# mrmod/h264decode

Hardware: AMD Instinct MI355X
Metric: 1080p Main CABAC frames/sec (higher is better)
Workload: dtype u8; 1 GPU; 1920x1080 Main CABAC IPPP GOP-30, 256 independent streams per GPU (32 distinct, each used 8 times), QP 28, 1 slice/frame, 1 ref; parallelism=streams sharded, no collective

## Files before the change

h264decode_amd/csrc/k_entropy.hip:

```cpp
#include <hip/hip_runtime.h>
#include "mi_kernels.h"
#include "k_common.h"

#ifndef MI_ENT_ISLICE_PRIO
#define MI_ENT_ISLICE_PRIO 0
#endif
#ifndef MI_ENT_MINWAVES
#define MI_ENT_MINWAVES 6
#endif
#ifndef MI_ENT_B
#define MI_ENT_B 0
#endif
#ifndef MI_ENT_FMO
#define MI_ENT_FMO MI_ENT_B
#endif
#ifndef MI_ENT_CABAC
#define MI_ENT_CABAC 0
#endif
#if MI_ENT_CABAC
#define ENT_CABAC(e) 1
#define IF_CAVLC(x) 0
#else
#define ENT_CABAC(e) ((e).cabac)
#define IF_CAVLC(x) (x)
#endif
#if MI_ENT_B
#define NL 2
#define MI_ENT_KERNEL k_entropy_b
#elif MI_ENT_FMO
#define NL 1
#define MI_ENT_KERNEL k_entropy_f
#elif MI_ENT_CABAC
#define NL 1
#define MI_ENT_KERNEL k_entropy_c
#else
#define NL 1
#define MI_ENT_KERNEL k_entropy
#endif
#define LANE (e.lane)
#define FI __device__ __forceinline__
#define LDS_SYNC()                                             \
    do {                                                       \
        __builtin_amdgcn_fence(__ATOMIC_RELEASE, "wavefront"); \
        __builtin_amdgcn_wave_barrier();                       \
        __builtin_amdgcn_fence(__ATOMIC_ACQUIRE, "wavefront"); \
    } while (0)

struct TopInfo {
    uint8_t type, t8x8, cbp, chroma_mode, cbf_dc;
    uint8_t dmask;
    uint16_t row;
    int8_t ipm[4];
    uint8_t nnz[8];
    int8_t ref[2][2];
    int16_t mv[NL][4][2];
    uint8_t mvd[NL][4][2];
};
#define TOP_DW (static_cast<int>(sizeof(TopInfo) / 4))
static_assert(sizeof(TopInfo) == (MI_ENT_B ? 72 : 48), "TopInfo layout");

struct Shared {
    uint8_t ctx[464];
#if !MI_ENT_CABAC
    uint8_t posmap[4][64];
#endif
    int16_t coef[MI_COEF_PER_MB];
    MbRec rec;
    TopInfo nb[4];
    int8_t ipm_c[32];
    uint8_t nnz_c[32];
    uint8_t nnzc_c[2][12];
    int8_t ref_c[NL][32];
    int8_t refi_c[NL][32];
    alignas(4) int16_t mv_c[NL][32][2];
    alignas(2) uint8_t mvd_c[NL][32][2];
    uint16_t parts[16];
    int8_t refs8[2][4];
    int8_t sub_type[4];
    uint8_t cur_cbf_dc, pad[3];
    int16_t ref_slot[NL][MI_MAX_REFS];
    uint32_t skip_tmpl[32];
    uint32_t role[64];
#if !MI_ENT_CABAC
    uint16_t vlc[MI_VLC_N];
#endif
    uint8_t coded[64];
#if MI_ENT_B
    uint32_t col[20];
    alignas(4) int16_t dmv[2][16][2];
    int8_t dref[2][4];
    int16_t dsf[MI_MAX_REFS];
#endif
};
#define GI(bx, by) (((by) + 1) * 6 + (bx) + 1)
enum { NB_LEFT = 0, NB_TL = 1, NB_TOP = 2 };

struct Ent {
    int lane;
    Shared *s;
    TopInfo *top;
    uint32_t pre_top;
    const DevTables *tab;
    const uint32_t *rbsp32;
    const SliceDesc *sd;
    const PicDesc *pd;
    MbRec *mbrec;
    int16_t *coefs;
    uint32_t *pool_head;
    uint32_t pool_blocks;
    uint32_t coef_cur, coef_end;
    uint64_t bitbuf;
    int bcnt;
    uint32_t wpos, wbase, rbsp_words;
    uint32_t win, winn, winx;
    uint32_t range, value;
    int avail;
    uint32_t ca, cb, wk;
    int wk_cat;
    uint32_t wk_c0;
    int wk_home;
    int wk_valid;
    uint32_t v_rlps, v_trans;
    uint32_t v_maps;
    uint32_t v_pos;
    uint32_t v_cat0, v_cat1;
    uint32_t v_qpc, v_refslot;
    uint32_t v_step;
    uint32_t aw, bw;
    int v_ipm;
    int qp, prev_dqp_nz, mbx, mby, cur_type, err;
    uint32_t qpw0, qpw1;
    int cabac, islice, wmb, hmb;
    int mono;
    int cip, t8x8_mode, cqp_off0, cqp_off1, nref;
    uint64_t mb_base;
#if MI_ENT_B
    int nref1, direct_spatial, d8inf, col_short, direct8;
    const uint32_t *col;
    uint32_t v_col;
    MbMv1 *mbmv1;
#endif
#if MI_ENT_STATS
    uint32_t bins;
    uint64_t tacc[4], tmark;
#endif
};
#if MI_ENT_STATS
#define MI_BINS(e) ((e).bins)
#define MI_COUNT_BIN(e) ((e).bins++)
#define MI_TT0(e) ((e).tmark = __builtin_readcyclecounter())
#define MI_TT(e, k) do { const uint64_t now_ = __builtin_readcyclecounter(); (e).tacc[k] += now_ - (e).tmark; (e).tmark = now_; } while (0)
#if MI_ENT_STATS == 4
#define MI_T0(e) ((void)0)
#define MI_T(e, k) ((void)0)
#define MI_R0(e) ((void)0)
#define MI_R(e, k) ((void)0)
#define MI_S(e, k) MI_TT(e, k)
#elif MI_ENT_STATS == 2
#define MI_T0(e) ((void)0)
#define MI_T(e, k) ((void)0)
#define MI_R0(e) ((void)0)
#define MI_R(e, k) ((void)0)
#define MI_R0(e) MI_TT0(e)
#define MI_R(e, k) MI_TT(e, k)
#else
#define MI_T0(e) MI_TT0(e)
#define MI_T(e, k) MI_TT(e, k)
#define MI_R0(e) ((void)0)
#define MI_R(e, k) ((void)0)
#endif
#else
#define MI_BINS(e) 0u
#define MI_COUNT_BIN(e) ((void)0)
#define MI_T0(e) ((void)0)
#define MI_T(e, k) ((void)0)
#define MI_R0(e) ((void)0)
#define MI_R(e, k) ((void)0)
#endif
#ifndef MI_S
#define MI_S(e, k) ((void)0)
#endif
#define RFL(x) __builtin_amdgcn_readfirstlane(x)
#define RDL(v, i) static_cast<uint32_t>(__builtin_amdgcn_readlane(static_cast<int>(v), static_cast<int>(i)))
extern "C" __device__ int mi_writelane(int val, int lane, int old) __asm("llvm.amdgcn.writelane.i32");

FI uint32_t cat_word0(int c) {
    const uint32_t maxnum[6] = {16, 15, 16, 4, 15, 64}, cbf[6] = {85, 89, 93, 97, 101, 64}, lim[6] = {4, 4, 4, 3, 4, 4}, pm[6] = {0, 1, 0, 3, 1, 2};
    const uint32_t nlast[6] = {15, 14, 15, 3, 14, 9};
    c = c < 6 ? c : 0;
    return maxnum[c] | (cbf[c] - 64) << 8 | lim[c] << 16 | pm[c] << 20 | nlast[c] << 24;
}
FI uint32_t cat_word1(int c, int field) {
    const uint32_t sig[6] = {105, 120, 134, 149, 152, 402}, last[6] = {166, 181, 195, 210, 213, 417}, ab[6] = {227, 237, 247, 257, 266, 426};
    const uint32_t sigf[6] = {277, 292, 306, 321, 324, 436}, lastf[6] = {338, 353, 367, 382, 385, 451};
    c = c < 6 ? c : 0;
    return (field ? sigf[c] : sig[c]) | (field ? lastf[c] : last[c]) << 10 | ab[c] << 20;
}

FI uint32_t load_win(const Ent &e, uint32_t base) {
    const uint32_t i = base + LANE;
    return i < e.rbsp_words ? __builtin_bswap32(e.rbsp32[i]) : 0u;
}
FI uint32_t fetch_word(Ent &e) {
    const uint32_t idx = e.wpos - e.wbase;
    e.wpos++;
    const uint32_t w0 = RDL(e.win, idx), w1 = RDL(e.winn, idx), w2 = RDL(e.winx, idx);
    return idx < 64 ? w0 : (idx < 128 ? w1 : w2);
}
FI void slide_window(Ent &e) {
    while (e.wpos - e.wbase >= 64) {
        e.win = e.winn, e.winn = e.winx;
        e.wbase += 64;
        e.winx = load_win(e, e.wbase + 128);
    }
}
FI uint32_t bitpos(const Ent &e) { return e.wpos * 32 - static_cast<uint32_t>(e.bcnt); }
FI void seek(Ent &e, uint32_t pos) {
// ... 718 lines not shown
            *reinterpret_cast<uint32_t *>(s->mv_c[0][g]) = w0, *reinterpret_cast<uint32_t *>(s->mv_c[1][g]) = w1;
        } else {
            *reinterpret_cast<uint32_t *>(s->dmv[0][l]) = w0, *reinterpret_cast<uint32_t *>(s->dmv[1][l]) = w1;
        }
        if (!((bx | by) & 1)) {
            if (commit)
                s->refs8[0][q] = static_cast<int8_t>(ref0), s->refs8[1][q] = static_cast<int8_t>(ref1);
            else
                s->dref[0][q] = static_cast<int8_t>(ref0), s->dref[1][q] = static_cast<int8_t>(ref1);
        }
    }
    LDS_SYNC();
}
FI void commit_direct(Ent &e, const int L, int q) {
    Shared *s = e.s;
    const int l = LANE, bx = l & 3, by = (l >> 2) & 3;
    if (l < 16 && (by >> 1) * 2 + (bx >> 1) == q) {
        const int g = GI(bx, by);
        s->ref_c[L][g] = s->dref[L][q];
        *reinterpret_cast<uint32_t *>(s->mv_c[L][g]) = *reinterpret_cast<const uint32_t *>(s->dmv[L][l]);
        if (!((bx | by) & 1)) s->refs8[L][q] = s->dref[L][q];
    }
    LDS_SYNC();
}
#endif

FI void read_ref_idx(Ent &e, const int L, int bx, int by, int w, int h, int nref) {
    Shared *s = e.s;
    int ref = 0;
    if (nref > 1) {
        if (ENT_CABAC(e)) {
            int ctx = (s->refi_c[L][GI(bx - 1, by)] > 0) + 2 * (s->refi_c[L][GI(bx, by - 1)] > 0);
            while (BIN_A(e, 54 + ctx)) {
                ctx = (ctx >> 2) + 4;
                if (++ref > 31) {
                    e.err = 3;
                    break;
                }
            }
        } else
            ref = IF_CAVLC(nref == 2 ? !get_bit(e) : static_cast<int>(get_ue(e)));
        if (ref >= nref || ref >= MI_MAX_REFS) e.err = 13, ref = 0;
    }
    {
        const int l = LANE, x = l & 3, y = (l >> 2) & 3;
        if (l < 16 && x >= bx && x < bx + w && y >= by && y < by + h) {
            s->refi_c[L][GI(x, y)] = static_cast<int8_t>(ref);
            if (!((x | y) & 1)) s->refs8[L][(y >> 1) * 2 + (x >> 1)] = static_cast<int8_t>(ref);
        }
        LDS_SYNC();
    }
}
FI void read_mv(Ent &e, const int L, int p) {
    Shared *s = e.s;
    const int bx = p & 3, by = (p >> 2) & 3, w = ((p >> 4) & 3) + 1, h = ((p >> 6) & 3) + 1, shape = (p >> 8) & 7;
    const int ref = s->refs8[L][(by >> 1) * 2 + (bx >> 1)];
    int d[2];
    for (int comp = 0; comp < 2; comp++) {
        int v;
        if (ENT_CABAC(e)) {
            const int sum = s->mvd_c[L][GI(bx - 1, by)][comp] + s->mvd_c[L][GI(bx, by - 1)][comp];
            const int base = comp ? 47 : 40;
            v = 0;
            if (BIN_A(e, base + (sum > 2) + (sum > 32))) {
                int ctx = base + 3;
                v = 1;
                while (v < 9 && BIN_A(e, ctx)) {
                    if (v < 4) ctx++;
                    v++;
                }
                if (v >= 9) v += cabac_egk(e, 3);
                if (cabac_bypass(e)) v = -v;
            }
        } else
            v = IF_CAVLC(get_se(e));
        d[comp] = v;
    }
    int px, py;
    predict_mv(e, L, bx, by, w, ref, shape, px, py);
    set_part(e, L, bx, by, w, h, ref, px + d[0], py + d[1], d[0], d[1]);
}

#if !MI_ENT_B
FI void pskip_fast(Ent &e) {
    Shared *s = e.s;
    int l = LANE;
    OPAQUE(l);
    const uint32_t *nbw = reinterpret_cast<const uint32_t *>(s->nb);
    const uint32_t tA = e.aw, tB = e.bw, tC = nbw[(NB_TOP + 1) * TOP_DW], tD = nbw[NB_TL * TOP_DW];
    const uint32_t rA = nbw[NB_LEFT * TOP_DW + 5], rB = nbw[NB_TOP * TOP_DW + 5], rC = nbw[(NB_TOP + 1) * TOP_DW + 5], rD = nbw[NB_TL * TOP_DW + 5];
    const uint32_t mA = nbw[NB_LEFT * TOP_DW + 6], mB = nbw[NB_TOP * TOP_DW + 6], mC = nbw[(NB_TOP + 1) * TOP_DW + 6], mD = nbw[NB_TL * TOP_DW + 9];
    auto ref_of = [](uint32_t t, uint32_t r, int byte) {
        const int type = static_cast<int>(t & 255u);
        return type == MBT_NONE ? -2 : (MB_IS_INTER(type) ? static_cast<int>(static_cast<int8_t>((r >> (8 * byte)) & 255u)) : -1);
    };
    auto mv_of = [](uint32_t t, uint32_t m) { return MB_IS_INTER(static_cast<int>(t & 255u)) ? m : 0u; };
    const int ra = ref_of(tA, rA, 0), rb = ref_of(tB, rB, 0);
    const bool c_ok = e.mbx + 1 < e.wmb && (tC & 255u) != MBT_NONE;
    const int rc = c_ok ? ref_of(tC, rC, 0) : ref_of(tD, rD, 1);
    const uint32_t va = mv_of(tA, mA), vb = mv_of(tB, mB), vc = c_ok ? mv_of(tC, mC) : mv_of(tD, mD);
    uint32_t mvw = 0;
    const bool zero = ra == -2 || rb == -2 || (ra == 0 && va == 0) || (rb == 0 && vb == 0);
    if (!zero) {
        const int na = ra == 0, nb_ = rb == 0, nc = rc == 0;
        if (na + nb_ + nc == 1)
            mvw = na ? va : (nb_ ? vb : vc);
        else {
            const int ax = static_cast<int16_t>(va & 0xffffu), ay = static_cast<int32_t>(va) >> 16, bx = static_cast<int16_t>(vb & 0xffffu), by = static_cast<int32_t>(vb) >> 16;
            const int cx = static_cast<int16_t>(vc & 0xffffu), cy = static_cast<int32_t>(vc) >> 16;
            mvw = (static_cast<uint32_t>(median3(ax, bx, cx)) & 0xffffu) | (static_cast<uint32_t>(median3(ay, by, cy)) << 16);
        }
    }
    e.cur_type = MBT_PSKIP;
    e.prev_dqp_nz = 0;
    if (l < TOP_DW) {
        const uint32_t row = MI_ENT_FMO ? static_cast<uint32_t>(e.mby + 1) << 16 : 0u;
        const uint32_t nw = l == 0 ? static_cast<uint32_t>(MBT_PSKIP) : (l == 1 ? row : (l == 2 ? 0xFFFFFFFFu : ((l >= 6 && l < 10) ? mvw : 0u)));
        uint32_t *tl = reinterpret_cast<uint32_t *>(&s->nb[NB_TL]), *tp = reinterpret_cast<uint32_t *>(&s->nb[NB_TOP]), *tr = reinterpret_cast<uint32_t *>(&s->nb[NB_TOP + 1]);
        const uint32_t old_top = tp[l], w1 = tr[l];
        tl[l] = old_top;
        tp[l] = w1;
        tr[l] = e.pre_top;
        reinterpret_cast<uint32_t *>(&s->nb[NB_LEFT])[l] = nw;
        reinterpret_cast<uint32_t *>(e.top + e.mbx)[l] = nw;
        e.pre_top = top_load(e, e.mbx + 3, l);
    } else if (l >= 32) {
        const int k = l - 32;
        const uint32_t t = s->skip_tmpl[k];
        const uint32_t w = k == 0 ? (static_cast<uint32_t>(MBT_PSKIP) | e.qpw0) : (k == 1 ? e.qpw1 : ((k >= 12 && k < 28) ? mvw : t));
        const uint64_t mbi = e.mb_base + static_cast<uint64_t>(e.mby) * e.wmb + e.mbx;
        reinterpret_cast<uint32_t *>(e.mbrec + mbi)[k] = w;
    }
    LDS_SYNC();
}
#endif

FI void decode_mb(Ent &e, int skipped) {
    Shared *s = e.s;
    MbRec &r = s->rec;
    const int cabac = ENT_CABAC(e), islice = e.islice;
    int cbp_luma = 0, cbp_chroma = 0, t8x8 = 0, i16mode = 0, chroma_mode = 0, has_coef = 0;
    int type, raw = 0, nparts = 0;
    const Nb a{e.aw}, b{e.bw};
    r.nzmask = 0;
#if MI_ENT_B
    int no_sub8 = 1;
    e.direct8 = 0;
#endif
    if (skipped) {
#if MI_ENT_B
        type = MBT_BSKIP;
        e.cur_type = type;
        e.direct8 = 15;
        direct_pred(e, 15, true);
#else
        type = MBT_PSKIP;
        e.cur_type = type;
        int mvx = 0, mvy = 0;
        int ra = s->ref_c[0][GI(-1, 0)], rb = s->ref_c[0][GI(0, -1)];
        bool zero = ra == -2 || rb == -2 || (ra == 0 && s->mv_c[0][GI(-1, 0)][0] == 0 && s->mv_c[0][GI(-1, 0)][1] == 0) ||
                    (rb == 0 && s->mv_c[0][GI(0, -1)][0] == 0 && s->mv_c[0][GI(0, -1)][1] == 0);
        if (!zero) predict_mv(e, 0, 0, 0, 4, 0, 0, mvx, mvy);
        set_part(e, 0, 0, 0, 4, 4, 0, mvx, mvy, 0, 0);
        s->refs8[0][0] = s->refs8[0][1] = s->refs8[0][2] = s->refs8[0][3] = 0;
#endif
        e.prev_dqp_nz = 0;
    } else {
        MI_S(e, 3);
        int intra_prefix = 1;
        if (cabac) {
#if MI_ENT_B
            {
                intra_prefix = 0;
                const int inc = (a.ok() && a.type() != MBT_BSKIP && a.type() != MBT_BDIRECT) + (b.ok() && b.type() != MBT_BSKIP && b.type() != MBT_BDIRECT);
                if (!BIN_A(e, 27 + inc))
                    raw = 0;
                else if (!BIN_A(e, 27 + 3))
                    raw = 1 + BINI_A(e, 27 + 5);
                else {
                    int bits = BINI_A(e, 27 + 4) << 3;
                    bits |= BINI_A(e, 27 + 5) << 2;
                    bits |= BINI_A(e, 27 + 5) << 1;
                    bits |= BINI_A(e, 27 + 5);
                    if (bits < 8)
                        raw = bits + 3;
                    else if (bits == 13)
                        intra_prefix = 1;
                    else if (bits == 14)
                        raw = 11;
                    else if (bits == 15)
                        raw = 22;
                    else
                        raw = ((bits << 1) | BINI_A(e, 27 + 5)) - 4;
                }
            }
#else
            if (!islice) {
                intra_prefix = BINI_A(e, 14);
                if (!intra_prefix) raw = BIN_A(e, 15) ? 2 - BINI_A(e, 17) : 3 * BINI_A(e, 16);
            }
#endif
            if (intra_prefix) {
                int base = islice ? 3 : (MI_ENT_B ? 32 : 17), it = 0, first;
                if (islice) {
                    int inc = (a.ok() && a.type() != MBT_I4x4 && a.type() != MBT_I8x8) + (b.ok() && b.type() != MBT_I4x4 && b.type() != MBT_I8x8);
                    first = BINI_A(e, base + inc);
                    base += 2;
                } else
                    first = BINI_A(e, base);
                if (first) {
                    if (cabac_terminate(e))
                        it = 25;
                    else {
                        it = 1 + 12 * BINI_A(e, base + 1);
                        if (BIN_A(e, base + 2)) it += 4 + 4 * BINI_A(e, base + 2 + islice);
                        it += 2 * BINI_A(e, base + 3 + islice);
                        it += BINI_A(e, base + 3 + 2 * islice);
                    }
                }
                raw = islice ? it : it + (MI_ENT_B ? 23 : 5);
            }
        } else
            raw = IF_CAVLC(static_cast<int>(get_ue(e)));
        const int it = islice ? raw : raw - (MI_ENT_B ? 23 : 5);
#if MI_ENT_B
        if (raw < 23)
            type = raw == 0 ? MBT_BDIRECT : MBT_B;
#else
        if (!islice && raw < 5)
            type = raw == 0 ? MBT_P16x16 : (raw == 1 ? MBT_P16x8 : (raw == 2 ? MBT_P8x16 : MBT_P8x8));
#endif
        else if (it == 0)
            type = MBT_I4x4;
        else if (it >= 1 && it <= 24) {
            type = MBT_I16x16;
            i16mode = (it - 1) & 3;
            cbp_chroma = ((it - 1) >> 2) % 3;
            cbp_luma = it >= 13 ? 15 : 0;
            if (cbp_chroma && e.mono) e.err = 25, cbp_chroma = 0;
        } else if (it == 25)
            type = MBT_IPCM;
        else {
            e.err = 20;
            type = MBT_I4x4;
        }
        e.cur_type = type;
        MI_S(e, 0);
        if (type == MBT_IPCM) {
            uint32_t pos = bitpos(e);
            if (cabac) pos -= static_cast<uint32_t>(RFL(e.avail));
            seek(e, (pos + 7) & ~7u);
            uint32_t *pcm = reinterpret_cast<uint32_t *>(s->coef);
            for (int i = 0; i < 96; i++) pcm[i] = (e.mono && i >= 64) ? 0x80808080u : __builtin_bswap32(get_bits(e, 32));
            if (cabac) cabac_start(e);
            for (int i = 0; i < 16; i++) {
                s->nnz_c[GI(i & 3, i >> 2)] = 16, s->ref_c[0][GI(i & 3, i >> 2)] = -1;
                if (MI_ENT_B) s->ref_c[NL - 1][GI(i & 3, i >> 2)] = -1;
            }
            for (int i = 0; i < 8; i++) s->nnzc_c[i >> 2][(((i >> 1) & 1) + 1) * 3 + (i & 1) + 1] = 16;
            s->cur_cbf_dc = 7;
            r.nzmask = 0xFFFF;
            cbp_luma = 15, cbp_chroma = 2;
            has_coef = 1;
            e.prev_dqp_nz = 0;
        } else {
            if (MB_IS_INTER(type)) {
#if MI_ENT_B
                if (type == MBT_BDIRECT) {
                    e.direct8 = 15;
                    direct_pred(e, 15, true);
                    no_sub8 = e.d8inf;
                } else {
                    int nref_parts;
                    if (raw <= 3) {
                        s->parts[0] = static_cast<uint16_t>(PART(0, 0, 4, 4, 0) | (raw << 11));
                        nparts = nref_parts = 1;
                    } else if (raw < 22) {
                        const int mm = b_pair_modes((raw - 4) >> 1), m0 = mm & 3, m1 = mm >> 2;
                        if (raw & 1)
                            s->parts[0] = static_cast<uint16_t>(PART(0, 0, 2, 4, 3) | (m0 << 11)), s->parts[1] = static_cast<uint16_t>(PART(2, 0, 2, 4, 4) | (m1 << 11));
                        else
                            s->parts[0] = static_cast<uint16_t>(PART(0, 0, 4, 2, 1) | (m0 << 11)), s->parts[1] = static_cast<uint16_t>(PART(0, 2, 4, 2, 2) | (m1 << 11));
                        nparts = nref_parts = 2;
                    } else {
                        nref_parts = 4;
                        for (int i = 0; i < 4; i++) {
                            int st;
                            if (cabac) {
                                if (!BIN_A(e, 36))
                                    st = 0;
                                else if (!BIN_A(e, 37))
                                    st = 1 + BINI_A(e, 39);
                                else {
                                    st = 3;
                                    int done = 0;
                                    if (BIN_A(e, 38)) {
                                        if (BIN_A(e, 39))
                                            st = 11 + BINI_A(e, 39), done = 1;
                                        else
                                            st += 4;
                                    }
                                    if (!done) {
                                        st += 2 * BINI_A(e, 39);
                                        st += BINI_A(e, 39);
                                    }
                                }
                            } else
                                st = IF_CAVLC(static_cast<int>(get_ue(e)));
                            if (st > 12) e.err = 21, st = 1;
                            s->sub_type[i] = static_cast<int8_t>(st);
                            const int md = b_sub_mode(st), shp = b_sub_shape(st);
                            const int bx = (i & 1) * 2, by = (i >> 1) * 2;
                            if (md == 0) {
                                e.direct8 |= 1 << i;
                                if (!e.d8inf) no_sub8 = 0;
                                s->parts[nparts++] = PART(bx, by, 2, 2, 0);
                            } else {
                                if (shp) no_sub8 = 0;
                                const int sw = (shp == 0 || shp == 1) ? 2 : 1, sh = (shp == 0 || shp == 2) ? 2 : 1;
                                for (int yy = 0; yy < 2; yy += sh)
                                    for (int xx = 0; xx < 2; xx += sw) s->parts[nparts++] = static_cast<uint16_t>(PART(bx + xx, by + yy, sw, sh, 0) | (md << 11));
                            }
                        }
                        if (e.direct8) direct_pred(e, e.direct8, false);
                    }
#pragma unroll
                    for (int L = 0; L < 2; L++)
                        for (int i = 0; i < nref_parts; i++) {
                            int bx, by, w, h, md;
                            if (raw == 22)
                                bx = (i & 1) * 2, by = (i >> 1) * 2, w = 2, h = 2, md = b_sub_mode(s->sub_type[i]);
                            else {
                                const int p = s->parts[i];
                                bx = p & 3, by = (p >> 2) & 3, w = ((p >> 4) & 3) + 1, h = ((p >> 6) & 3) + 1, md = p >> 11;
                            }
                            if ((md >> L) & 1) read_ref_idx(e, L, bx, by, w, h, L ? e.nref1 : e.nref);
                        }
#pragma unroll
                    for (int L = 0; L < 2; L++)
                        for (int i = 0; i < nparts; i++) {
                            const int p = s->parts[i], md = p >> 11;
                            const int bx = p & 3, by = (p >> 2) & 3;
                            if (md == 0)
                                commit_direct(e, L, (by >> 1) * 2 + (bx >> 1));
                            else if ((md >> L) & 1)
                                read_mv(e, L, p);
                            else
                                set_part(e, L, bx, by, ((p >> 4) & 3) + 1, ((p >> 6) & 3) + 1, -1, 0, 0, 0, 0);
                        }
                }
#else
                int nref_parts;
                if (type == MBT_P16x16) {
                    s->parts[0] = PART(0, 0, 4, 4, 0);
                    nparts = nref_parts = 1;
                } else if (type == MBT_P16x8) {
                    s->parts[0] = PART(0, 0, 4, 2, 1), s->parts[1] = PART(0, 2, 4, 2, 2);
                    nparts = nref_parts = 2;
                } else if (type == MBT_P8x16) {
                    s->parts[0] = PART(0, 0, 2, 4, 3), s->parts[1] = PART(2, 0, 2, 4, 4);
                    nparts = nref_parts = 2;
                } else {
                    nref_parts = 4;
                    for (int i = 0; i < 4; i++) {
                        int st;
                        if (cabac)
                            st = BIN_A(e, 21) ? 0 : (!BIN_A(e, 22) ? 1 : (BIN_A(e, 23) ? 2 : 3));
                        else
                            st = IF_CAVLC(static_cast<int>(get_ue(e)));
                        if (st > 3) e.err = 21, st = 0;
                        s->sub_type[i] = static_cast<int8_t>(st);
                        const int bx = (i & 1) * 2, by = (i >> 1) * 2;
                        const int sw = (st == 0 || st == 1) ? 2 : 1, sh = (st == 0 || st == 2) ? 2 : 1;
                        for (int yy = 0; yy < 2; yy += sh)
                            for (int xx = 0; xx < 2; xx += sw) s->parts[nparts++] = PART(bx + xx, by + yy, sw, sh, 0);
                    }
                }
                for (int i = 0; i < nref_parts; i++) {
                    int bx, by, w, h;
                    if (type == MBT_P8x8)
                        bx = (i & 1) * 2, by = (i >> 1) * 2, w = 2, h = 2;
                    else {
                        const int p = s->parts[i];
                        bx = p & 3, by = (p >> 2) & 3, w = ((p >> 4) & 3) + 1, h = ((p >> 6) & 3) + 1;
                    }
                    read_ref_idx(e, 0, bx, by, w, h, raw != 4 ? e.nref : 1);
                }
                for (int i = 0; i < nparts; i++) read_mv(e, 0, s->parts[i]);
#endif
            } else {
                if (type == MBT_I4x4 && e.t8x8_mode) {
                    t8x8 = cabac ? BINI_T8(e, (a.ok() && a.t8x8()) + (b.ok() && b.t8x8())) : IF_CAVLC(static_cast<int>(get_bit(e)));
                    if (t8x8) type = MBT_I8x8, e.cur_type = type;
                }
                if (type == MBT_I4x4 || type == MBT_I8x8) {
                    const int n = type == MBT_I8x8 ? 4 : 16;
                    for (int i = 0; i < n; i++) {
                        int bx, by;
                        if (n == 4)
                            bx = (i & 1) * 2, by = (i >> 1) * 2;
                        else
                            bx = (i & 1) + 2 * ((i >> 2) & 1), by = ((i >> 1) & 1) + 2 * (i >> 3);
                        const int pa = static_cast<int>(RDL(e.v_ipm, GI(bx - 1, by))), pb = static_cast<int>(RDL(e.v_ipm, GI(bx, by - 1)));
                        const int pred = (pa < -1 || pb < -1) ? 2 : (pa < pb ? pa : pb);
                        int mode = pred;
                        if (cabac) {
                            if (!BIN_B(e, 68)) {
                                int rem = 0;
                                for (int k = 0; k < 3; k++) rem |= BINI_B(e, 69) << k;
                                mode = rem < pred ? rem : rem + 1;
                            }
                        } else if (IF_CAVLC(!get_bit(e))) {
                            int rem = IF_CAVLC(static_cast<int>(get_bits(e, 3)));
                            mode = rem < pred ? rem : rem + 1;
                        }
                        const int g = GI(bx, by), d = LANE - g;
                        e.v_ipm = (d == 0 || (n == 4 && (d == 1 || d == 6 || d == 7))) ? mode : e.v_ipm;
                    }
                    if (LANE < 30) s->ipm_c[LANE] = static_cast<int8_t>(e.v_ipm);
                }
                if (e.mono)
                    chroma_mode = 0;
                else if (cabac) {
                    int inc = (a.ok() && MB_IS_INTRA(a.type()) && a.type() != MBT_IPCM && a.chroma_mode() != 0) +
                              (b.ok() && MB_IS_INTRA(b.type()) && b.type() != MBT_IPCM && b.chroma_mode() != 0);
                    chroma_mode = 0;
                    if (BIN_B(e, 64 + inc)) {
                        chroma_mode = 1;
                        while (chroma_mode < 3 && BIN_B(e, 67)) chroma_mode++;
                    }
                } else {
                    chroma_mode = IF_CAVLC(static_cast<int>(get_ue(e)));
                    if (chroma_mode > 3) e.err = 22, chroma_mode = 0;
                }
                if (LANE < 16) {
                    s->ref_c[0][GI(LANE & 3, LANE >> 2)] = -1;
                    if (MI_ENT_B) s->ref_c[NL - 1][GI(LANE & 3, LANE >> 2)] = -1;
                }
            }
            MI_S(e, MB_IS_INTER(type) ? 1 : 2);
            if (type != MBT_I16x16) {
                int cbp;
                if (cabac) {
                    const int cbp_a = a.ok() ? (a.type() == MBT_IPCM ? 0x2F : a.cbp()) : 0x0F;
                    const int cbp_b = b.ok() ? (b.type() == MBT_IPCM ? 0x2F : b.cbp()) : 0x0F;
                    cbp = 0;
                    for (int b8 = 0; b8 < 4; b8++) {
                        int ca = (b8 & 1) ? (cbp >> (b8 - 1)) & 1 : (cbp_a >> (b8 + 1)) & 1;
                        int cb = (b8 & 2) ? (cbp >> (b8 - 2)) & 1 : (cbp_b >> (b8 + 2)) & 1;
                        cbp |= BINI_B(e, 73 + (!ca) + 2 * (!cb)) << b8;
                    }
                    int ca = a.ok() && (a.type() == MBT_IPCM || (a.cbp() >> 4) != 0), cb = b.ok() && (b.type() == MBT_IPCM || (b.cbp() >> 4) != 0);
                    if (!e.mono && BIN_B(e, 77 + ca + 2 * cb)) {
                        ca = a.ok() && (a.type() == MBT_IPCM || (a.cbp() >> 4) == 2);
                        cb = b.ok() && (b.type() == MBT_IPCM || (b.cbp() >> 4) == 2);
                        cbp |= (1 + BINI_B(e, 77 + 4 + ca + 2 * cb)) << 4;
                    }
                } else {
                    uint32_t k = IF_CAVLC(get_ue(e));
                    if (k > (e.mono ? 15u : 47u)) e.err = 23, k = 0;
                    if (e.mono) k += 48;
                    cbp = IF_CAVLC(RFL(static_cast<int>(MB_IS_INTRA(type) ? e.tab->me_intra[k] : e.tab->me_inter[k])));
                }
                cbp_luma = cbp & 15, cbp_chroma = cbp >> 4;
                if (cbp_luma && e.t8x8_mode && MB_IS_INTER(type)) {
#if MI_ENT_B
                    const int all8 = no_sub8;
#else
                    int all8 = 1;
                    if (type == MBT_P8x8)
                        for (int i = 0; i < 4; i++) all8 &= s->sub_type[i] == 0;
#endif
                    if (all8) t8x8 = cabac ? BINI_T8(e, (a.ok() && a.t8x8()) + (b.ok() && b.t8x8())) : IF_CAVLC(static_cast<int>(get_bit(e)));
                }
            }
            if (cbp_luma || cbp_chroma || type == MBT_I16x16) {
                int dqp;
                if (cabac) {
                    int ctx = e.prev_dqp_nz ? 1 : 0, val = 0;
                    while (BIN_A(e, 60 + ctx)) {
                        ctx = 2 + (ctx >> 1);
                        if (++val > 104) {
                            e.err = 2;
                            break;
                        }
                    }
                    dqp = (val & 1) ? (val + 1) >> 1 : -((val + 1) >> 1);
                } else
                    dqp = IF_CAVLC(get_se(e));
                if (dqp < -26 || dqp > 25) e.err = 24, dqp = 0;
                e.prev_dqp_nz = dqp != 0;
                if (dqp) set_qp(e, (e.qp + dqp + 52) % 52);
                MI_S(e, 2);
                MI_T(e, 1);
                MI_R0(e);
                if (cabac)
                    parse_residual_cabac(e, cbp_luma, cbp_chroma, t8x8);
                else
                    IF_CAVLC((parse_residual_cavlc(e, cbp_luma, cbp_chroma, t8x8), 0));
                MI_R(e, 3);
                MI_T(e, 2);
                has_coef = 1;
            } else
                e.prev_dqp_nz = 0;
        }
    }
    MI_T(e, 1);
    const int qp_store = type == MBT_IPCM ? 0 : e.qp;
    r.type = static_cast<uint8_t>(type);
    r.t8x8 = static_cast<uint8_t>(t8x8);
    r.qp = static_cast<uint8_t>(qp_store);
    r.qpc[0] = static_cast<uint8_t>(RDL(e.v_qpc, min(max(qp_store + e.cqp_off0, 0), 51)));
    r.qpc[1] = static_cast<uint8_t>(RDL(e.v_qpc, min(max(qp_store + e.cqp_off1, 0), 51)));
    r.cbp = static_cast<uint8_t>(cbp_luma | (cbp_chroma << 4));
    r.chroma_mode = static_cast<uint8_t>(chroma_mode);
    r.i16mode = static_cast<uint8_t>(i16mode);
    {
        const int cip = e.cip;
        int av = 0;
        if (MB_IS_INTRA(type)) {
            const int td = s->nb[NB_TL].type, tc = nb_ok(e, NB_TOP + 1) ? s->nb[NB_TOP + 1].type : MBT_NONE;
            if (a.ok() && !(cip && MB_IS_INTER(a.type()))) av |= MI_AV_LEFT;
            if (b.ok() && !(cip && MB_IS_INTER(b.type()))) av |= MI_AV_TOP;
            if (td != MBT_NONE && !(cip && MB_IS_INTER(td))) av |= MI_AV_TOPLEFT;
            if (tc != MBT_NONE && !(cip && MB_IS_INTER(tc))) av |= MI_AV_TOPRIGHT;
        }
        r.avail = static_cast<uint8_t>(av);
    }
    LDS_SYNC();
    int l = LANE;
    OPAQUE(l);
    const int inter = MB_IS_INTER(type);
    uint32_t cmask = 0, coff = 0;
    if (has_coef) {
        bool nz = false;
        if (l < MI_COEF_BLOCKS) {
            const uint4 a = reinterpret_cast<const uint4 *>(s->coef)[2 * l], b = reinterpret_cast<const uint4 *>(s->coef)[2 * l + 1];
            nz = (a.x | a.y | a.z | a.w | b.x | b.y | b.z | b.w) != 0;
        }
        cmask = static_cast<uint32_t>(__builtin_amdgcn_ballot_w64(nz));
        if (type == MBT_IPCM) cmask = 0xFFFu;
// ... 69 lines not shown
    if (l < TOP_DW) {
        const uint32_t nw = reinterpret_cast<const uint32_t *>(tp)[l], w1 = reinterpret_cast<const uint32_t *>(&s->nb[NB_TOP + 1])[l];
        reinterpret_cast<uint32_t *>(e.top + e.mbx)[l] = nw;
        reinterpret_cast<uint32_t *>(&s->nb[NB_TOP])[l] = w1;
        reinterpret_cast<uint32_t *>(&s->nb[NB_TOP + 1])[l] = e.pre_top;
        e.pre_top = top_load(e, e.mbx + 3, l);
    }
    const uint64_t mbi = e.mb_base + static_cast<uint64_t>(e.mby) * e.wmb + e.mbx;
    if (l >= 32)
        reinterpret_cast<uint32_t *>(e.mbrec + mbi)[l - 32] = reinterpret_cast<const uint32_t *>(&r)[l - 32];
#if MI_ENT_B
    if (l < 16) reinterpret_cast<uint32_t *>(e.mbmv1 + mbi)[l] = inter ? *reinterpret_cast<const uint32_t *>(s->mv_c[1][GI(l & 3, l >> 2)]) : 0u;
#endif
    if (l < MI_COEF_BLOCKS && ((cmask >> l) & 1)) {
        uint4 *dst = reinterpret_cast<uint4 *>(e.coefs) + 2 * (static_cast<size_t>(coff) + __builtin_popcount(cmask & ((1u << l) - 1u)));
        dst[0] = reinterpret_cast<const uint4 *>(s->coef)[2 * l], dst[1] = reinterpret_cast<const uint4 *>(s->coef)[2 * l + 1];
        reinterpret_cast<uint4 *>(s->coef)[2 * l] = make_uint4(0, 0, 0, 0), reinterpret_cast<uint4 *>(s->coef)[2 * l + 1] = make_uint4(0, 0, 0, 0);
    }
    LDS_SYNC();
}

FI void fill_none(const Ent &e, int from, int to) {
    const int l = LANE;
    for (int a = from + (l >> 5); a < to; a += 2) reinterpret_cast<uint32_t *>(e.mbrec + e.mb_base + static_cast<uint64_t>(a))[l & 31] = 0u;
}

#if MI_ENT_B
extern "C" __global__ void __launch_bounds__(64) __attribute__((amdgpu_waves_per_eu(4, 8))) k_entropy_b(const SliceDesc *slices_, const PicDesc *pics, const uint8_t *bitstream, const DevTables *tab, MbRec *mbrec,
                                                           int16_t *coefs, uint32_t *pool_head, uint32_t pool_blocks, uint32_t *status_, uint32_t *toprows_, int wmb_max, uint32_t slice_base,
                                                           const BSliceExt *bexts, MbMv1 *mbmv1) {
#else
extern "C" __global__ void __launch_bounds__(64) __attribute__((amdgpu_waves_per_eu(MI_ENT_MINWAVES, 8))) MI_ENT_KERNEL(const SliceDesc *slices_, const PicDesc *pics, const uint8_t *bitstream, const DevTables *tab, MbRec *mbrec,
                                                           int16_t *coefs, uint32_t *pool_head, uint32_t pool_blocks, uint32_t *status_, uint32_t *toprows_, int wmb_max, uint32_t slice_base) {
#endif
    __shared__ Shared sh;
    const uint32_t slice_no = slice_base + blockIdx.x;
    const SliceDesc *slices = slices_ + slice_base;
    uint32_t *status = status_ + 8 * static_cast<size_t>(slice_base);
    uint32_t *toprows = toprows_ + static_cast<size_t>(slice_base) * wmb_max * TOP_DW;
    const uint64_t t_begin = wall_clock64();
    Ent e;
    e.lane = static_cast<int>(threadIdx.x);
    e.s = &sh;
#if MI_ENT_STATS
    e.bins = 0;
    for (int k = 0; k < 4; k++) e.tacc[k] = 0;
#endif
    e.top = reinterpret_cast<TopInfo *>(toprows + static_cast<size_t>(blockIdx.x) * wmb_max * TOP_DW);
    e.pre_top = 0;
    e.tab = tab;
    const SliceDesc *sd = &slices[blockIdx.x];
    const PicDesc *pd = &pics[sd->pic_idx];
    e.sd = sd, e.pd = pd;
    e.rbsp32 = reinterpret_cast<const uint32_t *>(bitstream + sd->rbsp_off);
    e.rbsp_words = RFL((sd->rbsp_size + 3) >> 2);
    e.mbrec = mbrec;
    e.coefs = coefs;
    e.pool_head = pool_head, e.pool_blocks = pool_blocks;
    e.coef_cur = e.coef_end = 0;
    e.err = 0;
    e.cabac = MI_ENT_CABAC ? 1 : RFL(static_cast<int>(pd->cabac));
    e.islice = RFL(static_cast<int>(sd->slice_type == 2));
#if MI_ENT_ISLICE_PRIO
    if (e.islice) __builtin_amdgcn_s_setprio(MI_ENT_ISLICE_PRIO);
#endif
    e.wmb = RFL(static_cast<int>(pd->wmb)), e.hmb = RFL(static_cast<int>(pd->hmb));
    e.cip = RFL(static_cast<int>(pd->cip)), e.t8x8_mode = RFL(static_cast<int>(pd->t8x8_mode));
    e.cqp_off0 = RFL(static_cast<int>(pd->cqp_off[0])), e.cqp_off1 = RFL(static_cast<int>(pd->cqp_off[1]));
    e.nref = RFL(static_cast<int>(sd->num_ref_idx_active));
    e.mb_base = (static_cast<uint64_t>(RFL(static_cast<uint32_t>(pd->mb_base >> 32))) << 32) | RFL(static_cast<uint32_t>(pd->mb_base));
    e.prev_dqp_nz = 0;
    e.range = 510, e.value = 0, e.avail = 0;
    e.mbx = e.mby = 0, e.cur_type = 0;
    const int l = LANE;
    {
        const uint8_t *rl = tab->range_lps[l];
        e.v_rlps = rl[0] | (rl[1] << 8) | (rl[2] << 16) | (static_cast<uint32_t>(rl[3]) << 24);
        e.v_trans = (static_cast<uint32_t>(tab->trans_lps[l]) ^ static_cast<uint32_t>(l)) | (l == 0 ? 0x80000040u : 0u) | (l < 62 ? 256u : 0u);
    }
    const uint8_t *scan4 = pd->field ? tab->fieldscan4 : tab->zigzag4, *scan8 = pd->field ? tab->fieldscan8 : tab->zigzag8;
    e.v_maps = (pd->field ? tab->sig8x8_field[l] : tab->sig8x8[l]) | (tab->last8x8[l] << 8) | (scan8[l] << 16) | (static_cast<uint32_t>(scan4[l & 15]) << 24);
    e.v_pos = scan4[l & 15] | (scan4[(l + 1) & 15] << 8) | (scan8[l] << 16) | (static_cast<uint32_t>(l) << 24);
    e.mono = RFL(static_cast<int>(pd->mono));
    e.v_cat0 = cat_word0(l), e.v_cat1 = cat_word1(l, pd->field != 0);
    e.v_qpc = tab->qpc[l < 52 ? l : 51];
    set_qp(e, RFL(static_cast<int>(sd->slice_qp)));
    e.v_step = step_word(l);
    e.aw = e.bw = 0;
    e.v_ipm = 0;
#if !MI_ENT_CABAC
    sh.posmap[0][l] = scan4[l & 15];
    sh.posmap[1][l] = scan4[(l + 1) & 15];
    sh.posmap[2][l] = scan8[l];
    sh.posmap[3][l] = static_cast<uint8_t>(l);
#endif
    if (l < MI_MAX_REFS) sh.ref_slot[0][l] = sd->ref_slot[l];
#if MI_ENT_B
    {
        const BSliceExt *bx = &bexts[sd->bext];
        if (l < MI_MAX_REFS) sh.ref_slot[1][l] = bx->ref_slot1[l], sh.dsf[l] = bx->dist_scale[l];
        e.nref1 = RFL(static_cast<int>(bx->num_ref_idx_l1_active));
        e.direct_spatial = RFL(static_cast<int>(bx->direct_spatial)), e.d8inf = RFL(static_cast<int>(bx->direct_8x8_inference));
        e.col_short = RFL(static_cast<int>(bx->col_short));
        e.col = reinterpret_cast<const uint32_t *>(bx->col);
        e.direct8 = 0, e.v_col = 0;
        e.mbmv1 = mbmv1;
    }
#endif
    {
        const int set = e.islice ? 0 : 1 + sd->cabac_init_idc;
        const uint8_t *src = tab->ctx_init[set][sd->slice_qp];
        e.ca = ctx_word(src[l]);
        e.cb = ctx_word(src[l < 61 ? 64 + l : 399 + (l - 61)]);
        e.wk = 0;
        e.wk_cat = -1, e.wk_c0 = 0, e.wk_home = 0, e.wk_valid = 0;
        for (int i = l; i < 464; i += 64) sh.ctx[i] = src[i];
    }
#if !MI_ENT_CABAC
    if (!pd->cabac)
        for (int i = l; i < MI_VLC_N / 2; i += 64) reinterpret_cast<uint32_t *>(sh.vlc)[i] = reinterpret_cast<const uint32_t *>(tab->vlc_c)[i];
#endif
    if (l < 32) reinterpret_cast<uint32_t *>(&sh.rec)[l] = 0;
    LDS_SYNC();
#if !MI_ENT_CABAC
    if (!pd->cabac) e.v_cat0 = l < 48 ? sh.vlc[MI_VLC_RUN + l] : 0u;
#endif
    if (l == 0) {
        sh.rec.dbf_idc = sd->dbf_idc;
        sh.rec.alpha_off = sd->alpha_off, sh.rec.beta_off = sd->beta_off;
        sh.rec.slice_in_pic = sd->slice_in_pic;
        sh.rec.slice_idx = slice_no;
        sh.rec.refslot1[0] = sh.rec.refslot1[1] = sh.rec.refslot1[2] = sh.rec.refslot1[3] = -1;
    }
    if (l < 32) {
        const uint32_t slot0 = static_cast<uint16_t>(sd->ref_slot[0]);
        sh.skip_tmpl[l] = l == 2 ? static_cast<uint32_t>(sd->dbf_idc) << 24
                                 : (l == 3 ? (static_cast<uint32_t>(static_cast<uint8_t>(sd->alpha_off)) | static_cast<uint32_t>(static_cast<uint8_t>(sd->beta_off)) << 8 |
                                              static_cast<uint32_t>(sd->slice_in_pic) << 16)
                                           : ((l == 9 || l == 10) ? (slot0 | slot0 << 16) : (l == 11 ? slice_no : (l >= 30 ? 0xFFFFFFFFu : 0u))));
    }
    for (int i = l; i < MI_COEF_PER_MB / 2; i += 64) reinterpret_cast<uint32_t *>(sh.coef)[i] = 0;
    sh.role[l] = build_role(l);
    for (int i = l; i < e.wmb * TOP_DW; i += 64) reinterpret_cast<uint32_t *>(e.top)[i] = 0;
    if (l < TOP_DW) reinterpret_cast<uint32_t *>(&sh.nb[NB_LEFT])[l] = 0, reinterpret_cast<uint32_t *>(&sh.nb[NB_TL])[l] = 0;
    if (l < 2 * TOP_DW) reinterpret_cast<uint32_t *>(&sh.nb[NB_TOP])[l] = 0;
    LDS_SYNC();
    {
        uint32_t pos = RFL(sd->data_bit_off);
        if (ENT_CABAC(e)) pos = (pos + 7) & ~7u;
        e.wbase = 0x80000000u;
        seek(e, pos);
        if (ENT_CABAC(e)) cabac_start(e);
    }
    const int total = min(e.wmb * e.hmb, RFL(static_cast<int>(sd->end_mb)));
#if !MI_ENT_CABAC
    const uint32_t stop_bit = RFL(sd->stop_bit);
#endif
    int addr = RFL(static_cast<int>(sd->first_mb));
    const bool fmo = MI_ENT_FMO && RFL(static_cast<int>(pd->fmo)) != 0;
    bool consecutive = false;
    if (!fmo) fill_none(e, RFL(static_cast<int>(sd->fill_from)), min(addr, total));
    e.mbx = addr % e.wmb, e.mby = addr / e.wmb;
#if MI_ENT_CABAC
    int more = 1;
#else
    int more = 1, skip_state = 0 , pending = 0;
#endif
    int n_mbs = 0;
    while (more && !e.err) {
        if (addr >= total) {
            e.err = 30;
            break;
        }
        if (fmo) {
            asm volatile("s_waitcnt vmcnt(0)" ::: "memory");
            if (!consecutive && l < TOP_DW) {
                reinterpret_cast<uint32_t *>(&sh.nb[NB_LEFT])[l] = 0;
                reinterpret_cast<uint32_t *>(&sh.nb[NB_TL])[l] = e.mbx > 0 ? top_load(e, e.mbx - 1, l) : 0u;
            }
            if (l < 2 * TOP_DW) reinterpret_cast<uint32_t *>(&sh.nb[NB_TOP])[l] = top_load(e, e.mbx + l / TOP_DW, l % TOP_DW);
            LDS_SYNC();
            if (l < 3 && sh.nb[NB_TL + l].row != static_cast<uint16_t>(e.mby)) sh.nb[NB_TL + l].type = MBT_NONE;
            LDS_SYNC();
        } else if (e.mbx == 0 || n_mbs == 0) {
            if (l < TOP_DW) reinterpret_cast<uint32_t *>(&sh.nb[NB_LEFT])[l] = 0, reinterpret_cast<uint32_t *>(&sh.nb[NB_TL])[l] = 0;
            asm volatile("s_waitcnt vmcnt(0)" ::: "memory");
            if (l < 2 * TOP_DW) reinterpret_cast<uint32_t *>(&sh.nb[NB_TOP])[l] = top_load(e, e.mbx + l / TOP_DW, l % TOP_DW);
            if (l < TOP_DW) e.pre_top = top_load(e, e.mbx + 2, l);
            LDS_SYNC();
        }
        OPAQUE(e.lane);
        slide_window(e);
        MI_T0(e);
#if MI_ENT_B
        e.v_col = (e.col && l < 20) ? e.col[static_cast<size_t>(addr) * 20 + l] : ((l >= 16 && l < 19) ? 0xFFFFFFFFu : 0u);
#endif
        e.aw = RFL(*reinterpret_cast<const uint32_t *>(&sh.nb[NB_LEFT])), e.bw = RFL(*reinterpret_cast<const uint32_t *>(&sh.nb[NB_TOP]));
        int skipped = 0;
        if (!e.islice) {
            if (ENT_CABAC(e)) {
                const Nb a{e.aw}, b{e.bw};
                const int skip_type = MI_ENT_B ? MBT_BSKIP : MBT_PSKIP;
                skipped = BINI_A(e, (MI_ENT_B ? 24 : 11) + (a.ok() && a.type() != skip_type) + (b.ok() && b.type() != skip_type));
            }
#if !MI_ENT_CABAC
            else {
                if (skip_state == 0) {
                    pending = static_cast<int>(get_ue(e));
                    if (pending > total - addr) e.err = 31, pending = 0;
                    if (pending > 0) skip_state = 1;
                }
                if (skip_state == 1) {
                    skipped = 1;
                    pending--;
                }
            }
#endif
        }
#if !MI_ENT_B
        if (skipped) {
            MI_T(e, 1);
            pskip_fast(e);
        } else
#endif
        {
            MI_T(e, 1);
            fill_caches(e);
            MI_T(e, 0);
            decode_mb(e, skipped);
        }
        MI_T(e, 3);
        if (e.err) break;
        n_mbs++;
        if (ENT_CABAC(e))
            more = !cabac_terminate(e);
#if !MI_ENT_CABAC
        else if (skipped) {
            if (pending == 0) {
                more = bitpos(e) < stop_bit;
                skip_state = 2;
            }
        } else {
            more = bitpos(e) < stop_bit;
            skip_state = 0;
        }
#endif
        if (fmo) {
            const uint8_t *sgmap = bitstream + RFL(e.pd->sgmap_off);
            const int sgroup = RFL(static_cast<int>(sgmap[RFL(static_cast<int>(e.sd->first_mb))]));
            const uint32_t inv_wmb = RFL(e.pd->inv_wmb);
            int next = total;
            for (int base = addr + 1; base < total; base += 64) {
                const int i = base + l;
                const unsigned long long m = __builtin_amdgcn_ballot_w64(i < total && sgmap[i] == sgroup);
                if (m) {
                    next = base + __builtin_ctzll(m);
                    break;
                }
            }
            consecutive = next == addr + 1 && e.mbx + 1 < e.wmb;
            addr = next;
            e.mby = static_cast<int>(MI_MB_ROW(static_cast<uint32_t>(addr), inv_wmb)), e.mbx = addr - e.mby * e.wmb;
        } else {
            addr++;
            if (++e.mbx == e.wmb) e.mbx = 0, e.mby++;
        }
    }
    if (!fmo) fill_none(e, addr, total);
    if (l == 0) {
        status[8 * blockIdx.x] = static_cast<uint32_t>(e.err);
        status[8 * blockIdx.x + 1] = static_cast<uint32_t>(n_mbs);
        status[8 * blockIdx.x + 2] = static_cast<uint32_t>(wall_clock64() - t_begin);
        status[8 * blockIdx.x + 3] = MI_BINS(e);
#if MI_ENT_STATS
        for (int k = 0; k < 4; k++) status[8 * blockIdx.x + 4 + k] = static_cast<uint32_t>(e.tacc[k] >> 4);
#if MI_ENT_STATS == 3
        status[8 * blockIdx.x + 4] = static_cast<uint32_t>(t_begin), status[8 * blockIdx.x + 5] = static_cast<uint32_t>(wall_clock64());
#endif
#endif
    }
}
```

Measured before the change: 30430 frames/s.

## Add fast path for P16x16 macroblocks in CABAC entropy decode

Adds a specialized CABAC path for P_L0_16x16 macroblocks. It reads mb_type early, then decodes ref_idx, mvd and cbp directly and predicts the motion vector from the cached neighbours. When cbp is zero it writes the neighbour and record words straight away, the same way the P-skip path does, and skips fill_caches and decode_mb. Otherwise it hands the pre-decoded values to decode_mb, which no longer re-reads mb_type, ref, mvd or cbp. It also packs slice constants (nref, cip, mono, t8x8) into a scalar word that is unpacked each macroblock. The aim is to cut per-macroblock overhead for common P16x16 blocks, at the cost of duplicated prediction logic that could diverge from the general path.

```diff
diff --git a/h264decode_amd/csrc/k_entropy.hip b/h264decode_amd/csrc/k_entropy.hip
--- a/h264decode_amd/csrc/k_entropy.hip
+++ b/h264decode_amd/csrc/k_entropy.hip
@@ -16,6 +16,12 @@
 #endif
 #ifndef MI_ENT_CABAC
 #define MI_ENT_CABAC 0
+#endif
+#ifndef MI_ENT_P16FAST
+#define MI_ENT_P16FAST (MI_ENT_CABAC && !MI_ENT_B && !MI_ENT_FMO)
+#endif
+#ifndef MI_ENT_SC
+#define MI_ENT_SC MI_ENT_P16FAST
 #endif
 #if MI_ENT_CABAC
 #define ENT_CABAC(e) 1
@@ -133,6 +139,9 @@
     int cabac, islice, wmb, hmb;
     int mono;
     int cip, t8x8_mode, cqp_off0, cqp_off1, nref;
+#if MI_ENT_SC
+    uint32_t sc;
+#endif
     uint64_t mb_base;
 #if MI_ENT_B
     int nref1, direct_spatial, d8inf, col_short, direct8;
@@ -1017,11 +1026,8 @@
 }
 
 #if !MI_ENT_B
-FI void pskip_fast(Ent &e) {
-    Shared *s = e.s;
-    int l = LANE;
-    OPAQUE(l);
-    const uint32_t *nbw = reinterpret_cast<const uint32_t *>(s->nb);
+FI uint32_t nb_mv_pred(const Ent &e, const int ref, const bool skip) {
+    const uint32_t *nbw = reinterpret_cast<const uint32_t *>(e.s->nb);
     const uint32_t tA = e.aw, tB = e.bw, tC = nbw[(NB_TOP + 1) * TOP_DW], tD = nbw[NB_TL * TOP_DW];
     const uint32_t rA = nbw[NB_LEFT * TOP_DW + 5], rB = nbw[NB_TOP * TOP_DW + 5], rC = nbw[(NB_TOP + 1) * TOP_DW + 5], rD = nbw[NB_TL * TOP_DW + 5];
     const uint32_t mA = nbw[NB_LEFT * TOP_DW + 6], mB = nbw[NB_TOP * TOP_DW + 6], mC = nbw[(NB_TOP + 1) * TOP_DW + 6], mD = nbw[NB_TL * TOP_DW + 9];
@@ -1030,14 +1036,15 @@
         return type == MBT_NONE ? -2 : (MB_IS_INTER(type) ? static_cast<int>(static_cast<int8_t>((r >> (8 * byte)) & 255u)) : -1);
     };
     auto mv_of = [](uint32_t t, uint32_t m) { return MB_IS_INTER(static_cast<int>(t & 255u)) ? m : 0u; };
-    const int ra = ref_of(tA, rA, 0), rb = ref_of(tB, rB, 0);
+    int ra = ref_of(tA, rA, 0), rb = ref_of(tB, rB, 0);
     const bool c_ok = e.mbx + 1 < e.wmb && (tC & 255u) != MBT_NONE;
-    const int rc = c_ok ? ref_of(tC, rC, 0) : ref_of(tD, rD, 1);
-    const uint32_t va = mv_of(tA, mA), vb = mv_of(tB, mB), vc = c_ok ? mv_of(tC, mC) : mv_of(tD, mD);
+    int rc = c_ok ? ref_of(tC, rC, 0) : ref_of(tD, rD, 1);
+    uint32_t va = mv_of(tA, mA), vb = mv_of(tB, mB), vc = c_ok ? mv_of(tC, mC) : mv_of(tD, mD);
     uint32_t mvw = 0;
-    const bool zero = ra == -2 || rb == -2 || (ra == 0 && va == 0) || (rb == 0 && vb == 0);
+    const bool zero = skip && (ra == -2 || rb == -2 || (ra == 0 && va == 0) || (rb == 0 && vb == 0));
+    if (!skip && rb == -2 && rc == -2 && ra != -2) rb = rc = ra, vb = vc = va;
     if (!zero) {
-        const int na = ra == 0, nb_ = rb == 0, nc = rc == 0;
+        const int na = ra == ref, nb_ = rb == ref, nc = rc == ref;
         if (na + nb_ + nc == 1)
             mvw = na ? va : (nb_ ? vb : vc);
         else {
@@ -1046,6 +1053,13 @@
             mvw = (static_cast<uint32_t>(median3(ax, bx, cx)) & 0xffffu) | (static_cast<uint32_t>(median3(ay, by, cy)) << 16);
         }
     }
+    return mvw;
+}
+FI void pskip_fast(Ent &e) {
+    Shared *s = e.s;
+    int l = LANE;
+    OPAQUE(l);
+    const uint32_t mvw = nb_mv_pred(e, 0, true);
     e.cur_type = MBT_PSKIP;
     e.prev_dqp_nz = 0;
     if (l < TOP_DW) {
@@ -1070,7 +1084,107 @@
 }
 #endif
 
-FI void decode_mb(Ent &e, int skipped) {
+FI int read_cbp_cabac(Ent &e, const Nb a, const Nb b) {
+    const int cbp_a = a.ok() ? (a.type() == MBT_IPCM ? 0x2F : a.cbp()) : 0x0F;
+    const int cbp_b = b.ok() ? (b.type() == MBT_IPCM ? 0x2F : b.cbp()) : 0x0F;
+    int cbp = 0;
+    for (int b8 = 0; b8 < 4; b8++) {
+        int ca = (b8 & 1) ? (cbp >> (b8 - 1)) & 1 : (cbp_a >> (b8 + 1)) & 1;
+        int cb = (b8 & 2) ? (cbp >> (b8 - 2)) & 1 : (cbp_b >> (b8 + 2)) & 1;
+        cbp |= BINI_B(e, 73 + (!ca) + 2 * (!cb)) << b8;
+    }
+    int ca = a.ok() && (a.type() == MBT_IPCM || (a.cbp() >> 4) != 0), cb = b.ok() && (b.type() == MBT_IPCM || (b.cbp() >> 4) != 0);
+    if (!e.mono && BIN_B(e, 77 + ca + 2 * cb)) {
+        ca = a.ok() && (a.type() == MBT_IPCM || (a.cbp() >> 4) == 2);
+        cb = b.ok() && (b.type() == MBT_IPCM || (b.cbp() >> 4) == 2);
+        cbp |= (1 + BINI_B(e, 77 + 4 + ca + 2 * cb)) << 4;
+    }
+    return cbp;
+}
+
+#if MI_ENT_P16FAST
+FI bool p16_fast(Ent &e, uint32_t &pk, uint32_t &mvw_out) {
+    Shared *s = e.s;
+    int l = LANE;
+    OPAQUE(l);
+    const uint32_t *nbw = reinterpret_cast<const uint32_t *>(s->nb);
+    const Nb a{e.aw}, b{e.bw};
+    int ref = 0;
+    if (e.nref > 1) {
+        const int ia = MB_IS_INTER(a.type()) && static_cast<int8_t>(nbw[NB_LEFT * TOP_DW + 5] & 255u) > 0;
+        const int ib = MB_IS_INTER(b.type()) && static_cast<int8_t>(nbw[NB_TOP * TOP_DW + 5] & 255u) > 0;
+        int ctx = ia + 2 * ib;
+        while (BIN_A(e, 54 + ctx)) {
+            ctx = (ctx >> 2) + 4;
+            if (++ref > 31) {
+                e.err = 3;
+                break;
+            }
+        }
+        if (ref >= e.nref || ref >= MI_MAX_REFS) e.err = 13, ref = 0;
+    }
+    const uint32_t mvd_ab = (nbw[NB_LEFT * TOP_DW + 10] & 0xffffu) | nbw[NB_TOP * TOP_DW + 10] << 16;
+    int dx = 0, dy = 0;
+#pragma nounroll
+    for (int comp = 0; comp < 2; comp++) {
+        const int sum = static_cast<int>(((mvd_ab >> (8 * comp)) & 255u) + ((mvd_ab >> (16 + 8 * comp)) & 255u));
+        const int base = comp ? 47 : 40;
+        int v = 0;
+        if (BIN_A(e, base + (sum > 2) + (sum > 32))) {
+            int ctx = base + 3;
+            v = 1;
+            while (v < 9 && BIN_A(e, ctx)) {
+                if (v < 4) ctx++;
+                v++;
+            }
+            if (v >= 9) v += cabac_egk(e, 3);
+            if (cabac_bypass(e)) v = -v;
+        }
+        if (comp)
+            dy = v;
+        else
+            dx = v;
+    }
+    const int cbp = read_cbp_cabac(e, a, b);
+    const uint32_t pw = nb_mv_pred(e, ref, false);
+    const int mvx = static_cast<int16_t>(pw & 0xffffu) + dx, mvy = (static_cast<int32_t>(pw) >> 16) + dy;
+    const uint32_t mvw = (static_cast<uint32_t>(mvx) & 0xffffu) | (static_cast<uint32_t>(mvy) << 16);
+    const uint32_t refb = static_cast<uint32_t>(ref);
+    const uint32_t amvd = static_cast<uint32_t>(min(abs(dx), 255)) | static_cast<uint32_t>(min(abs(dy), 255)) << 8;
+    if (cbp) {
+        pk = refb | static_cast<uint32_t>(cbp) << 8 | amvd << 16, mvw_out = mvw;
+        return false;
+    }
+    MI_T(e, 1);
+    e.cur_type = MBT_P16x16;
+    e.prev_dqp_nz = 0;
+    const uint32_t mvdw = amvd * 0x10001u;
+    if (l < TOP_DW) {
+        const uint32_t nw = l == 0 ? static_cast<uint32_t>(MBT_P16x16)
+                                   : (l == 2 ? 0xFFFFFFFFu : (l == 5 ? refb * 0x101u : ((l >= 6 && l < 10) ? mvw : (l >= 10 ? mvdw : 0u))));
+        uint32_t *tl = reinterpret_cast<uint32_t *>(&s->nb[NB_TL]), *tp = reinterpret_cast<uint32_t *>(&s->nb[NB_TOP]), *tr = reinterpret_cast<uint32_t *>(&s->nb[NB_TOP + 1]);
+        const uint32_t old_top = tp[l], w1 = tr[l];
+        tl[l] = old_top;
+        tp[l] = w1;
+        tr[l] = e.pre_top;
+        reinterpret_cast<uint32_t *>(&s->nb[NB_LEFT])[l] = nw;
+        reinterpret_cast<uint32_t *>(e.top + e.mbx)[l] = nw;
+        e.pre_top = top_load(e, e.mbx + 3, l);
+    } else if (l >= 32) {
+        const int k = l - 32;
+        const uint32_t slot = static_cast<uint16_t>(s->ref_slot[0][ref]);
+        const uint32_t t = s->skip_tmpl[k];
+        const uint32_t w = k == 0 ? (static_cast<uint32_t>(MBT_P16x16) | e.qpw0)
+                                  : (k == 1 ? e.qpw1 : (k == 8 ? refb * 0x01010101u : ((k == 9 || k == 10) ? slot * 0x10001u : ((k >= 12 && k < 28) ? mvw : t))));
+        const uint64_t mbi = e.mb_base + static_cast<uint64_t>(e.mby) * e.wmb + e.mbx;
+        reinterpret_cast<uint32_t *>(e.mbrec + mbi)[k] = w;
+    }
+    LDS_SYNC();
+    return true;
+}
+#endif
+
+FI void decode_mb(Ent &e, int skipped, const int pre, const uint32_t pk, const uint32_t mvw) {
     Shared *s = e.s;
     MbRec &r = s->rec;
     const int cabac = ENT_CABAC(e), islice = e.islice;
@@ -1130,10 +1244,14 @@
                 }
             }
 #else
+#if MI_ENT_P16FAST
+            if (!islice) intra_prefix = pre < 0, raw = pre < 0 ? 0 : pre;
+#else
             if (!islice) {
                 intra_prefix = BINI_A(e, 14);
                 if (!intra_prefix) raw = BIN_A(e, 15) ? 2 - BINI_A(e, 17) : 3 * BINI_A(e, 16);
             }
+#endif
 #endif
             if (intra_prefix) {
                 int base = islice ? 3 : (MI_ENT_B ? 32 : 17), it = 0, first;
@@ -1285,6 +1403,13 @@
                         }
                 }
 #else
+#if MI_ENT_P16FAST
+                if (type == MBT_P16x16) {
+                    const int ref = static_cast<int>(pk & 255u);
+                    if (LANE < 4) s->refs8[0][LANE] = static_cast<int8_t>(ref);
+                    set_part(e, 0, 0, 0, 4, 4, ref, static_cast<int16_t>(mvw & 0xffffu), static_cast<int32_t>(mvw) >> 16, static_cast<int>((pk >> 16) & 255u), static_cast<int>(pk >> 24));
+                } else {
+#endif
                 int nref_parts;
                 if (type == MBT_P16x16) {
                     s->parts[0] = PART(0, 0, 4, 4, 0);
@@ -1322,6 +1447,9 @@
                     read_ref_idx(e, 0, bx, by, w, h, raw != 4 ? e.nref : 1);
                 }
                 for (int i = 0; i < nparts; i++) read_mv(e, 0, s->parts[i]);
+#if MI_ENT_P16FAST
+                }
+#endif
 #endif
             } else {
                 if (type == MBT_I4x4 && e.t8x8_mode) {
@@ -1376,22 +1504,14 @@
             MI_S(e, MB_IS_INTER(type) ? 1 : 2);
             if (type != MBT_I16x16) {
                 int cbp;
-                if (cabac) {
-                    const int cbp_a = a.ok() ? (a.type() == MBT_IPCM ? 0x2F : a.cbp()) : 0x0F;
-                    const int cbp_b = b.ok() ? (b.type() == MBT_IPCM ? 0x2F : b.cbp()) : 0x0F;
-                    cbp = 0;
-                    for (int b8 = 0; b8 < 4; b8++) {
-                        int ca = (b8 & 1) ? (cbp >> (b8 - 1)) & 1 : (cbp_a >> (b8 + 1)) & 1;
-                        int cb = (b8 & 2) ? (cbp >> (b8 - 2)) & 1 : (cbp_b >> (b8 + 2)) & 1;
-                        cbp |= BINI_B(e, 73 + (!ca) + 2 * (!cb)) << b8;
-                    }
-                    int ca = a.ok() && (a.type() == MBT_IPCM || (a.cbp() >> 4) != 0), cb = b.ok() && (b.type() == MBT_IPCM || (b.cbp() >> 4) != 0);
-                    if (!e.mono && BIN_B(e, 77 + ca + 2 * cb)) {
-                        ca = a.ok() && (a.type() == MBT_IPCM || (a.cbp() >> 4) == 2);
-                        cb = b.ok() && (b.type() == MBT_IPCM || (b.cbp() >> 4) == 2);
-                        cbp |= (1 + BINI_B(e, 77 + 4 + ca + 2 * cb)) << 4;
-                    }
-                } else {
+#if MI_ENT_P16FAST
+                if (type == MBT_P16x16)
+                    cbp = static_cast<int>((pk >> 8) & 255u);
+                else
+#endif
+                if (cabac)
+                    cbp = read_cbp_cabac(e, a, b);
+                else {
                     uint32_t k = IF_CAVLC(get_ue(e));
                     if (k > (e.mono ? 15u : 47u)) e.err = 23, k = 0;
                     if (e.mono) k += 48;
@@ -1627,6 +1747,9 @@
     e.v_maps = (pd->field ? tab->sig8x8_field[l] : tab->sig8x8[l]) | (tab->last8x8[l] << 8) | (scan8[l] << 16) | (static_cast<uint32_t>(scan4[l & 15]) << 24);
     e.v_pos = scan4[l & 15] | (scan4[(l + 1) & 15] << 8) | (scan8[l] << 16) | (static_cast<uint32_t>(l) << 24);
     e.mono = RFL(static_cast<int>(pd->mono));
+#if MI_ENT_SC
+    e.sc = static_cast<uint32_t>(e.nref) | static_cast<uint32_t>(e.cip != 0) << 8 | static_cast<uint32_t>(e.mono != 0) << 9 | static_cast<uint32_t>(e.t8x8_mode != 0) << 10;
+#endif
     e.v_cat0 = cat_word0(l), e.v_cat1 = cat_word1(l, pd->field != 0);
     e.v_qpc = tab->qpc[l < 52 ? l : 51];
     set_qp(e, RFL(static_cast<int>(sd->slice_qp)));
@@ -1735,6 +1858,13 @@
             LDS_SYNC();
         }
         OPAQUE(e.lane);
+#if MI_ENT_SC
+        {
+            uint32_t sc = e.sc;
+            asm volatile("" : "+s"(sc));
+            e.nref = static_cast<int>(sc & 63u), e.cip = static_cast<int>((sc >> 8) & 1u), e.mono = static_cast<int>((sc >> 9) & 1u), e.t8x8_mode = static_cast<int>((sc >> 10) & 1u);
+        }
+#endif
         slide_window(e);
         MI_T0(e);
 #if MI_ENT_B
@@ -1742,6 +1872,9 @@
 #endif
         e.aw = RFL(*reinterpret_cast<const uint32_t *>(&sh.nb[NB_LEFT])), e.bw = RFL(*reinterpret_cast<const uint32_t *>(&sh.nb[NB_TOP]));
         int skipped = 0;
+#if MI_ENT_P16FAST
+        int pre = -1;
+#endif
         if (!e.islice) {
             if (ENT_CABAC(e)) {
                 const Nb a{e.aw}, b{e.bw};
@@ -1761,6 +1894,9 @@
                 }
             }
 #endif
+#if MI_ENT_P16FAST
+            if (!skipped && !BIN_A(e, 14)) pre = BIN_A(e, 15) ? 2 - BINI_A(e, 17) : 3 * BINI_A(e, 16);
+#endif
         }
 #if !MI_ENT_B
         if (skipped) {
@@ -1769,10 +1905,22 @@
         } else
 #endif
         {
-            MI_T(e, 1);
-            fill_caches(e);
-            MI_T(e, 0);
-            decode_mb(e, skipped);
+#if MI_ENT_P16FAST
+            uint32_t pk = 0, mvw = 0;
+            if (pre != 0 || !p16_fast(e, pk, mvw)) {
+                MI_T(e, 1);
+                fill_caches(e);
+                MI_T(e, 0);
+                decode_mb(e, skipped, pre, pk, mvw);
+            }
+#else
+            {
+                MI_T(e, 1);
+                fill_caches(e);
+                MI_T(e, 0);
+                decode_mb(e, skipped, -1, 0u, 0u);
+            }
+#endif
         }
         MI_T(e, 3);
         if (e.err) break;
```

New measurement: 30670 frames/s, median of 6. About the same (+0.8%).
